# SebastianAment/CovarianceFunctions.jl

Measured on AMD Instinct MI355X. Metric: Gramian MVMs/sec, dense EQ kernel, n=131072, d=3, fp32 (+ achieved HBM GB/s in roofline.hbm_*), higher is better.
Workload: dtype f32; 1 GPU; EQ dense Gramian mul!, d=3 n=131072 fp32 (BASELINE.json configs[1]); x ~ N(0, I_3), a ~ N(0,1), alpha=1, beta=0, y == x; all n*m entries evaluated; points/a/b resident in HBM; n=131072, d=3, kernel=EQ, parallelism=1 GPU

## Files before the change

### covariancefunctions.jl_amd/csrc/dense_mfma_eq.hpp

```cpp
#pragma once
#include "dense_mfma.hpp"

namespace covgram {

__global__ __launch_bounds__(256) void mfma_pack_kernel(const float* __restrict__ Y, int64_t m, int32_t d, uint4* __restrict__ PB,
                                                        float* __restrict__ EF, int32_t K2, float g, const float* __restrict__ Cn, int32_t fmt) {
    const int64_t e = (int64_t)blockIdx.x * blockDim.x + threadIdx.x;
    const int64_t ntile = (m + 31) / 32;
    if (e >= ntile * K2 * 64) return;
    const int l = (int)(e & 63);
    const int64_t q = e >> 6;
    const int mm = (int)(q % K2);
    const int64_t T = q / K2;
    const int64_t j = 32 * T + (l & 31);
    if (fmt == 1) {
        const int c0 = 4 * mm + 2 * (l >> 5);
        const bool nl = mm == 0 && (l >> 5) == 0;
        uint4 frag = make_uint4(0, 0, 0, 0);
        if (j < m) {
            const float ya = c0 < d ? g * (Y[j * (int64_t)d + c0] - Cn[c0]) : 0.0f;
            const float yb = c0 + 1 < d ? g * (Y[j * (int64_t)d + c0 + 1] - Cn[c0 + 1]) : 0.0f;
            unsigned a1, a2, b1, b2;
            split2h(ya, a1, a2);
            split2h(yb, b1, b2);
            frag = make_uint4(a1 | (a2 << 16), a1 | (b1 << 16), b2 | (b1 << 16), 0u);
            if (nl) {
                double ny = 0.0;
                for (int cc = 0; cc < d; ++cc) { const double yc = (double)(g * (Y[j * (int64_t)d + cc] - Cn[cc])); ny = __builtin_fma(yc, yc, ny); }
                const double hn = -0.5 * ny, k = __builtin_ceil(hn);
                frag.w = F16_ONE | (f16_bits((float)k) << 16);
                EF[j] = __builtin_amdgcn_exp2f((float)(hn - k));
            }
        } else if (nl) {
            EF[j] = 0.0f;
        }
        PB[e] = frag;
        return;
    }
    const int c = 2 * mm + (l >> 5);
    uint4 frag = make_uint4(0, 0, 0, 0);
    const bool norm_lane = (d & 1) ? (c == d) : (c == 0);
    if (j < m) {
        if (c < d) {
            const float yt = g * (Y[j * (int64_t)d + c] - Cn[c]);
            unsigned y1, y2, y3;
            split3(yt, y1, y2, y3);
            frag = make_uint4(y1 | (y2 << 16), y1 | (y3 << 16), y2 | (y1 << 16), y3 | (y2 << 16));
        }
        if (norm_lane) {
            double ny = 0.0;
            for (int cc = 0; cc < d; ++cc) { const double yc = (double)(g * (Y[j * (int64_t)d + cc] - Cn[cc])); ny = __builtin_fma(yc, yc, ny); }
            const NormSplit sp = norm_split(ny);
            if (d & 1) frag = make_uint4(BF16_ONE | (sp.kbits << 16), 0, 0, 0);
            else frag.w = BF16_ONE | (sp.kbits << 16);
            EF[j] = sp.ef;
        }
    } else if (norm_lane) {
        EF[j] = 0.0f;
    }
    PB[e] = frag;
}

__global__ __launch_bounds__(256) void mfma_pack_w_kernel(const float* __restrict__ A, const float* __restrict__ EF, float* __restrict__ W,
                                                          int64_t m, int64_t mpad) {
    const int64_t j = (int64_t)blockIdx.x * blockDim.x + threadIdx.x;
    if (j < mpad) W[j] = j < m ? A[j] * EF[j] : 0.0f;
}

template <int K2, int RT, int WPB = 1, int LDS = 0, int STAMP = 0, int FMT = 0>
__global__ __launch_bounds__(64 * WPB) __attribute__((amdgpu_waves_per_eu(LDS == 1 ? (RT == 4 ? 2 : K2 <= 2 ? 4 : 3) : 1, LDS == 1 ? (RT == 4 ? 2 : K2 <= 2 ? 4 : 3) : 8))) void dense_mfma_eq_kernel(const float* __restrict__ X, int64_t n, int32_t d,
                                                           const uint4* __restrict__ PB, const float* __restrict__ W, int64_t ntile,
                                                           float* __restrict__ out, int64_t npad, int64_t tchunk, float g,
                                                           float alpha, float beta, int32_t final_store, const float* __restrict__ Cn,
                                                           unsigned long long* __restrict__ stamps, unsigned* __restrict__ tickets,
                                                           float* __restrict__ yfinal, const float* __restrict__ EF, int64_t mcols) {
    const int l = threadIdx.x & 63, t = l & 31, h = l >> 5;
    const int64_t i0 = ((int64_t)blockIdx.x * WPB + (threadIdx.x >> 6)) * (32 * RT);
    Frag a[RT][K2];
    float er[RT];
#pragma unroll
    for (int r = 0; r < RT; ++r) {
        int64_t row = i0 + 32 * r + t;
        if (row >= n) row = n - 1;
        er[r] = eq_row_fragments_fmt<K2, FMT>(X + row * (int64_t)d, Cn, d, g, h, a[r]);
    }

    unsigned long long st_c0 = 0, st_r0 = 0;
    if constexpr (STAMP) { st_c0 = __builtin_amdgcn_s_memtime(); st_r0 = __builtin_amdgcn_s_memrealtime(); }
    const int64_t T0 = (int64_t)blockIdx.y * tchunk;
    const int64_t T1 = (T0 + tchunk < ntile) ? (T0 + tchunk) : ntile;
    typedef float f32x2 __attribute__((ext_vector_type(2)));
    f32x2 acc2[RT][8];
#pragma unroll
    for (int r = 0; r < RT; ++r)
#pragma unroll
        for (int v = 0; v < 8; ++v) acc2[r][v] = (f32x2){0.0f, 0.0f};

    const uint4* __restrict__ pbase = PB + (T0 * K2) * 64;
    const float* __restrict__ wbase = W + T0 * 32;
    const int nt = (int)(T1 - T0);
    auto weight = [&](int tc) {
        if (EF == nullptr) return wbase[tc * 32 + t];
        const int64_t j = (T0 + tc) * 32 + t;
        return j < mcols ? W[j] * EF[j] : 0.0f;
    };
    auto load_tile = [&](int ti, Frag (&f)[K2], float& w) {
        const int tc = ti < nt ? ti : nt - 1;
#pragma unroll
        for (int mm = 0; mm < K2; ++mm) f[mm].u = pbase[(tc * K2 + mm) * 64 + l];
        w = weight(tc);
    };
    auto process = [&](const Frag (&f)[K2], float w) {
        f32x16 D[RT];
#pragma unroll
        for (int r = 0; r < RT; ++r) {
            D[r] = (f32x16){0, 0, 0, 0, 0, 0, 0, 0, 0, 0, 0, 0, 0, 0, 0, 0};
#pragma unroll
            for (int mm = 0; mm < K2; ++mm) D[r] = eq_mma<FMT>(a[r][mm], f[mm], D[r]);
        }
#pragma unroll
        for (int r = 0; r < RT; ++r)
#pragma unroll
            for (int v = 0; v < 16; ++v) D[r][v] = __builtin_amdgcn_exp2f(D[r][v]);
#pragma unroll
        for (int r = 0; r < RT; ++r)
#pragma unroll
            for (int v = 0; v < 8; ++v) {
                if constexpr (K2 <= 2) acc2[r][v] = __builtin_elementwise_fma((f32x2){w, w}, (f32x2){D[r][2 * v], D[r][2 * v + 1]}, acc2[r][v]);
                else { acc2[r][v][0] = __builtin_fmaf(w, D[r][2 * v], acc2[r][v][0]); acc2[r][v][1] = __builtin_fmaf(w, D[r][2 * v + 1], acc2[r][v][1]); }
            }
    };
    if constexpr (LDS == 2) {
        static_assert(RT == 1, "split-tile staging is built for one row tile per wave");
        __shared__ uint4 tfA[K2][64], tfB[K2][64];
        __shared__ float twA[32], twB[32];
        typedef __attribute__((address_space(1))) const void* gptr_t;
        typedef __attribute__((address_space(3))) void* lptr_t;
        const int wv = __builtin_amdgcn_readfirstlane(threadIdx.x >> 6);
        float gw = 0.0f, ge = 1.0f;
#define CG_DMA2(tile, TF)                                                                       \
        {                                                                                       \
            const int ti_ = (tile);                                                             \
            const int tc_ = ti_ < nt ? ti_ : nt - 1;                                            \
            _Pragma("unroll") for (int q = 0; q < (K2 + WPB - 1) / WPB; ++q) {                  \
                const int mm = wv + q * WPB;                                                    \
                if (mm < K2) __builtin_amdgcn_global_load_lds((gptr_t)(pbase + (tc_ * K2 + mm) * 64 + l), (lptr_t)&TF[mm][0], 16, 0, 0); \
            }                                                                                   \
            if (wv == 0) {                                                                      \
                if (EF == nullptr) gw = ti_ < nt ? wbase[tc_ * 32 + t] : 0.0f;                  \
                else {                                                                          \
                    const int64_t j_ = (T0 + tc_) * 32 + t;                                     \
                    const bool in_ = ti_ < nt && j_ < mcols;                                    \
                    gw = in_ ? W[j_] : 0.0f; ge = in_ ? EF[j_] : 0.0f;                          \
                }                                                                               \
            }                                                                                   \
        }
#define CG_TILE2(TF, TW)                                                                        \
        {                                                                                       \
            f32x16 D = {0, 0, 0, 0, 0, 0, 0, 0, 0, 0, 0, 0, 0, 0, 0, 0};                        \
            Frag f_[K2];                                                                        \
            _Pragma("unroll") for (int mm = 0; mm < K2; ++mm) f_[mm].u = TF[mm][l];             \
            const float w = TW[t];                                                              \
            _Pragma("unroll") for (int mm = 0; mm < K2; ++mm) D = eq_mma<FMT>(a[0][mm], f_[mm], D); \
            _Pragma("unroll") for (int v = 0; v < 16; ++v) D[v] = __builtin_amdgcn_exp2f(D[v]); \
            _Pragma("unroll") for (int v = 0; v < 8; ++v) { acc2[0][v][0] = __builtin_fmaf(w, D[2 * v], acc2[0][v][0]); acc2[0][v][1] = __builtin_fmaf(w, D[2 * v + 1], acc2[0][v][1]); } \
        }
        CG_DMA2(0, tfA)
        if (wv == 0 && h == 0) twA[t] = gw * ge;
        __syncthreads();
        for (int ti = 0; ti < nt; ti += 2) {
            CG_DMA2(ti + 1, tfB)
            CG_TILE2(tfA, twA)
            if (wv == 0 && h == 0) twB[t] = gw * ge;
            __syncthreads();
            if (ti + 1 >= nt) break;
            CG_DMA2(ti + 2, tfA)
            CG_TILE2(tfB, twB)
            if (wv == 0 && h == 0) twA[t] = gw * ge;
            __syncthreads();
        }
#undef CG_DMA2
#undef CG_TILE2
    } else if constexpr (LDS == 1) {
        __shared__ uint4 sfA[WPB][K2][64], sfB[WPB][K2][64];
        __shared__ float swA[WPB][32], swB[WPB][32];
        typedef __attribute__((address_space(1))) const void* gptr_t;
        typedef __attribute__((address_space(3))) void* lptr_t;
        const int wv = __builtin_amdgcn_readfirstlane(threadIdx.x >> 6);
        const int nstage = (nt + WPB - 1) / WPB;
        float gw, ge = 1.0f;
#define CG_DMA(stage, SF)                                                                       \
        {                                                                                       \
            const int ti_ = (stage) * WPB + wv;                                                 \
            const int tc_ = ti_ < nt ? ti_ : nt - 1;                                            \
            _Pragma("unroll") for (int mm = 0; mm < K2; ++mm)                                   \
                __builtin_amdgcn_global_load_lds((gptr_t)(pbase + (tc_ * K2 + mm) * 64 + l), (lptr_t)&SF[wv][mm][0], 16, 0, 0); \
            if (EF == nullptr) gw = ti_ < nt ? wbase[tc_ * 32 + t] : 0.0f;    \
            else {                                                                              \
                const int64_t j_ = (T0 + tc_) * 32 + t;                                         \
                const bool in_ = ti_ < nt && j_ < mcols;                                        \
                gw = in_ ? W[j_] : 0.0f; ge = in_ ? EF[j_] : 0.0f;                              \
            }                                                                                   \
        }
#define CG_STAGE(SF, SW)                                                                        \
        _Pragma("unroll 1") for (int k = 0; k < WPB; k += 2) {                                  \
            Frag f0[K2], f1[K2];                                                                \
            _Pragma("unroll") for (int mm = 0; mm < K2; ++mm) f0[mm].u = SF[k][mm][l];          \
            const float w0 = SW[k][t];                                                          \
            _Pragma("unroll") for (int mm = 0; mm < K2; ++mm) f1[mm].u = SF[k + 1][mm][l];      \
            const float w1 = SW[k + 1][t];                                                      \
            process(f0, w0);                                                                    \
            process(f1, w1);                                                                    \
        }
        CG_DMA(0, sfA)
        if (h == 0) swA[wv][t] = gw * ge;
        __syncthreads();
        for (int st = 0; st < nstage; st += 2) {
            CG_DMA(st + 1 < nstage ? st + 1 : st, sfB)
            CG_STAGE(sfA, swA)
            if (h == 0) swB[wv][t] = gw * ge;
            __syncthreads();
            if (st + 1 >= nstage) break;
            CG_DMA(st + 2 < nstage ? st + 2 : st + 1, sfA)
            CG_STAGE(sfB, swB)
            if (h == 0) swA[wv][t] = gw * ge;
            __syncthreads();
        }
#undef CG_DMA
#undef CG_STAGE
    } else {
    Frag f0[K2], f1[K2];
    float w0, w1;
    load_tile(0, f0, w0);
    for (int ti = 0; ti < nt; ti += 2) {
        load_tile(ti + 1, f1, w1);
        process(f0, w0);
        load_tile(ti + 2, f0, w0);
        if (ti + 1 < nt) process(f1, w1);
    }
    }

    if constexpr (STAMP) {
        const unsigned long long c1 = __builtin_amdgcn_s_memtime(), r1 = __builtin_amdgcn_s_memrealtime();
        if (threadIdx.x == 0) {
            unsigned long long* o = stamps + 4 * ((size_t)blockIdx.y * gridDim.x + blockIdx.x);
            o[0] = st_c0; o[1] = st_r0; o[2] = c1; o[3] = r1;
        }
    }
    const int vsel = (t & 3) + 4 * (t >> 3);
#pragma unroll
    for (int r = 0; r < RT; ++r) {
        float tot = 0.0f;
#pragma unroll
        for (int v = 0; v < 16; ++v) {
            float s = acc2[r][v >> 1][v & 1];
            s += __shfl_xor(s, 1); s += __shfl_xor(s, 2); s += __shfl_xor(s, 4); s += __shfl_xor(s, 8); s += __shfl_xor(s, 16);
            tot = (vsel == v) ? s : tot;
        }
        const int64_t i = i0 + 32 * r + t;
        if (((t >> 2) & 1) != h || i >= n) continue;
        const float res = er[r] * tot;
        if (final_store) {
            float v = alpha * res;
            if (beta != 0.0f) v = __builtin_fmaf(beta, out[i], v);
            out[i] = v;
        } else {
            slab_store(out + (int64_t)blockIdx.y * npad + i, res, tickets != nullptr);
        }
    }
    if (!final_store && tickets != nullptr) {
        if (!last_arrival(tickets + blockIdx.x, gridDim.y)) return;
        const int64_t r0 = (int64_t)blockIdx.x * (WPB * 32 * RT);
        for (int idx = threadIdx.x; idx < WPB * 32 * RT; idx += 64 * WPB) {
            const int64_t i = r0 + idx;
            if (i >= n) continue;
            float v = alpha * ordered_split_sum<float>(out + i, npad, (int)gridDim.y);
            if (beta != 0.0f) v = __builtin_fmaf(beta, yfinal[i], v);
            yfinal[i] = v;
        }
    }
}

__global__ __launch_bounds__(256) void mfma_pack_gen_kernel(const float* __restrict__ Y, int64_t m, int32_t d, const float* __restrict__ A,
                                                            int64_t lda, int32_t nrhs, int32_t c0, uint4* __restrict__ PB,
                                                            float* __restrict__ W, int32_t K2, int32_t NR, float g, int32_t iso,
                                                            const float* __restrict__ Cn, int32_t fmt) {
    const int64_t e = (int64_t)blockIdx.x * blockDim.x + threadIdx.x;
    const int64_t ntile = (m + 31) / 32;
    if (e >= ntile * K2 * 64) return;
    const int l = (int)(e & 63);
    const int64_t q = e >> 6;
    const int mm = (int)(q % K2);
    const int64_t T = q / K2;
    const int64_t j = 32 * T + (l & 31);
    const int c = 2 * mm + (l >> 5);
    uint4 frag = make_uint4(0, 0, 0, 0);
    if (fmt == 1) {
        if (j < m) {
            float ny = 0.0f;
            for (int cc = 0; cc < d; ++cc) { const float yc = g * (Y[j * (int64_t)d + cc] - Cn[cc]); ny = __builtin_fmaf(yc, yc, ny); }
            unsigned sl[6] = {0, 0, 0, 0, 0, 0};
            for (int w = 0; w < 2; ++w) {
                const int qq = 4 * mm + 2 * (l >> 5) + w;
                if (qq < d) { unsigned y1, y2; split2h(-2.0f * (g * (Y[j * (int64_t)d + qq] - Cn[qq])), y1, y2); sl[3 * w] = y1; sl[3 * w + 1] = y2; sl[3 * w + 2] = y1; }
                else if (qq == d) { sl[3 * w] = sl[3 * w + 1] = sl[3 * w + 2] = F16_ONE; }
                else if (qq == d + 1) { const Norm16 nn = norm16(ny); sl[3 * w] = nn.k; sl[3 * w + 1] = nn.f1; sl[3 * w + 2] = nn.f2; }
            }
            frag = make_uint4(sl[0] | (sl[1] << 16), sl[2] | (sl[3] << 16), sl[4] | (sl[5] << 16), 0u);
        }
    } else
    if (j < m) {
        if (c < d) {
            const float yt = iso ? -2.0f * (g * (Y[j * (int64_t)d + c] - Cn[c])) : g * Y[j * (int64_t)d + c];
            unsigned y1, y2, y3;
            split3(yt, y1, y2, y3);
            frag = make_uint4(y1 | (y2 << 16), y1 | (y3 << 16), y2 | (y1 << 16), y3 | (y2 << 16));
        } else if (iso && c == d) {
            float ny = 0.0f;
            for (int cc = 0; cc < d; ++cc) { const float yc = g * (Y[j * (int64_t)d + cc] - Cn[cc]); ny = __builtin_fmaf(yc, yc, ny); }
            unsigned n1, n2, n3;
            split3(ny, n1, n2, n3);
            frag = make_uint4(BF16_ONE | (BF16_ONE << 16), BF16_ONE | (n1 << 16), n2 | (n3 << 16), 0);
        }
    }
    PB[e] = frag;
    if (mm == 0 && l < 32)
        for (int cr = 0; cr < NR; ++cr) W[(T * NR + cr) * 32 + l] = (j < m && c0 + cr < nrhs) ? A[j + (int64_t)(c0 + cr) * lda] : 0.0f;
}

__global__ __launch_bounds__(256) void mfma_pack_rhs_kernel(const float* __restrict__ A, int64_t lda, int32_t nrhs, int32_t c0, int64_t m,
                                                            float* __restrict__ AP, int32_t NB) {
    const int64_t e = (int64_t)blockIdx.x * blockDim.x + threadIdx.x;
    const int64_t ntile = (m + 31) / 32;
    if (e >= ntile * NB * 64 * 16) return;
    const int v = (int)(e & 15), l = (int)((e >> 4) & 63);
    const int64_t q = e >> 10;
    const int b = (int)(q % NB);
    const int64_t T = q / NB;
    const int64_t j = 32 * T + 8 * (v >> 2) + 4 * (l >> 5) + (v & 3);
    const int c = c0 + 32 * b + (l & 31);
    AP[e] = (j < m && c < nrhs) ? A[j + (int64_t)c * lda] : 0.0f;
}

}
```

Before: 731.4 MVM/s.

## Stage two column tiles per wave per LDS buffer in K2=1 EQ kernel

```diff
diff --git a/covariancefunctions.jl_amd/csrc/dense_mfma_eq.hpp b/covariancefunctions.jl_amd/csrc/dense_mfma_eq.hpp
--- a/covariancefunctions.jl_amd/csrc/dense_mfma_eq.hpp
+++ b/covariancefunctions.jl_amd/csrc/dense_mfma_eq.hpp
@@ -67,6 +67,8 @@
     if (j < mpad) W[j] = j < m ? A[j] * EF[j] : 0.0f;
 }
 
+constexpr int EQ_STAGE_TPW = 2;
+
 template <int K2, int RT, int WPB = 1, int LDS = 0, int STAMP = 0, int FMT = 0>
 __global__ __launch_bounds__(64 * WPB) __attribute__((amdgpu_waves_per_eu(LDS == 1 ? (RT == 4 ? 2 : K2 <= 2 ? 4 : 3) : 1, LDS == 1 ? (RT == 4 ? 2 : K2 <= 2 ? 4 : 3) : 8))) void dense_mfma_eq_kernel(const float* __restrict__ X, int64_t n, int32_t d,
                                                            const uint4* __restrict__ PB, const float* __restrict__ W, int64_t ntile,
@@ -181,6 +183,57 @@
         }
 #undef CG_DMA2
 #undef CG_TILE2
+    } else if constexpr (LDS == 1 && K2 == 1) {
+        constexpr int TPW = EQ_STAGE_TPW, NT = WPB * TPW;
+        __shared__ uint4 sfA[NT][64], sfB[NT][64];
+        __shared__ float swA[NT][32], swB[NT][32];
+        typedef __attribute__((address_space(1))) const void* gptr_t;
+        typedef __attribute__((address_space(3))) void* lptr_t;
+        const int wv = __builtin_amdgcn_readfirstlane(threadIdx.x >> 6);
+        const int nstage = (nt + NT - 1) / NT;
+        const bool fused = EF != nullptr;
+        float gw[TPW], ge[TPW];
+        bool ok[TPW];
+#define CG_DMA(stage, SF)                                                                       \
+        _Pragma("unroll") for (int q = 0; q < TPW; ++q) {                                       \
+            const int sl_ = q * WPB + wv;                                                       \
+            const int ti_ = (stage) * NT + sl_;                                                 \
+            const int tc_ = ti_ < nt ? ti_ : nt - 1;             \
+            __builtin_amdgcn_global_load_lds((gptr_t)(pbase + tc_ * 64 + l), (lptr_t)&SF[sl_][0], 16, 0, 0); \
+            const int64_t j_ = (T0 + tc_) * 32 + t;                                             \
+            ok[q] = ti_ < nt && j_ < mcols;                                                     \
+            gw[q] = W[fused && j_ >= mcols ? mcols - 1 : j_];                                   \
+            ge[q] = (fused ? EF : W)[j_];                                                       \
+        }
+#define CG_WEIGHTS(SW)                                                                          \
+        if (h == 0) { _Pragma("unroll") for (int q = 0; q < TPW; ++q) SW[q * WPB + wv][t] = ok[q] ? (fused ? gw[q] * ge[q] : gw[q]) : 0.0f; }
+#define CG_STAGE(SF, SW)                                                                        \
+        _Pragma("unroll 1") for (int k = 0; k < NT; k += 2) {                                   \
+            Frag f0[1], f1[1];                                                                  \
+            f0[0].u = SF[k][l];                                                                 \
+            const float w0 = SW[k][t];                                                          \
+            f1[0].u = SF[k + 1][l];                                                             \
+            const float w1 = SW[k + 1][t];                                                      \
+            process(f0, w0);                                                                    \
+            process(f1, w1);                                                                    \
+        }
+        CG_DMA(0, sfA)
+        CG_WEIGHTS(swA)
+        __syncthreads();
+        for (int st = 0; st < nstage; st += 2) {
+            CG_DMA(st + 1 < nstage ? st + 1 : st, sfB)
+            CG_STAGE(sfA, swA)
+            CG_WEIGHTS(swB)
+            __syncthreads();
+            if (st + 1 >= nstage) break;
+            CG_DMA(st + 2 < nstage ? st + 2 : st + 1, sfA)
+            CG_STAGE(sfB, swB)
+            CG_WEIGHTS(swA)
+            __syncthreads();
+        }
+#undef CG_DMA
+#undef CG_WEIGHTS
+#undef CG_STAGE
     } else if constexpr (LDS == 1) {
         __shared__ uint4 sfA[WPB][K2][64], sfB[WPB][K2][64];
         __shared__ float swA[WPB][32], swB[WPB][32];
```

Result: no change. 733.3 MVM/s, median of 3 (+0.3%).
